# k-flouris/cmf

Hardware: AMD Instinct MI355X
Metric: log-density evals/sec (JtJ-cholesky path), MNIST D=784 d=64 bs=512 (higher is better)
Workload: dtype f32 (3x3 tangent convs as bf16x3 split MFMA, fp32 accumulate); 1 GPU; C3: MNIST-shaped (1,28,28) uint8-range + U[0,1) noise, non-square flow d=64, cholesky J^T J log-det + g_ij off-diagonal L1 + reconstruction, eval/no_grad; per_gpu_batch=512, global_batch=512, D=784, latent_dimension=64, parallelism=dp1

## Files before the change

cmf_amd/_lib.py:

```python
import ctypes as C
import os
import threading

_HERE = os.path.dirname(os.path.abspath(__file__))
LIB_PATH = os.path.join(_HERE, "libcmf_amd.so")

F_NONE, F_RELU, F_TANH, F_RAW, F_SELF_RELU, F_RELU_BITS = 0, 1, 2, 3, 4, 5
O_NONE, O_TANH, O_STANH = 0, 1, 2

_fp = C.c_void_p
_ll = C.c_longlong
_i = C.c_int
_f = C.c_float
_d = C.c_double


class ConvTangentArgs(C.Structure):
    _fields_ = [("x", _fp), ("x_np", _ll), ("x_ci", _ll), ("x_px", _ll),
                ("f", _fp), ("f_np", _ll), ("f_ci", _ll), ("f_px", _ll), ("fmode", _i),
                ("w", _fp),
                ("y", _fp), ("y_np", _ll), ("y_co", _ll), ("y_px", _ll),
                ("r", _fp), ("r_np", _ll), ("r_co", _ll), ("r_px", _ll),
                ("np", _i), ("cin", _i), ("cout", _i), ("H", _i), ("W", _i), ("nc", _i), ("taps", _i),
                ("bias", _fp), ("f_group", _i), ("x_sl", _ll), ("y_sl", _ll), ("r_sl", _ll),
                ("fo", _fp), ("fo_np", _ll), ("fo_co", _ll), ("fo_px", _ll), ("fomode", _i),
                ("mask_out", _fp), ("mask_np", _ll), ("amax_in", _fp), ("amax_out", _fp), ("live", _i),
                ("ymask", _fp), ("ymask_np", _ll),
                ("head_w", _fp), ("head_cout", _i), ("head_a", _fp), ("head_a_np", _ll), ("head_a_c", _ll), ("head_a_px", _ll),
                ("head_y", _fp), ("head_y_np", _ll), ("head_y_co", _ll), ("head_y_px", _ll),
                ("seed", _fp), ("seed_np", _ll), ("seed_col", _ll), ("seed_w", _fp)]


class ConvPrimalArgs(C.Structure):
    _fields_ = [("x", _fp), ("x_b", _ll), ("x_c", _ll), ("x_px", _ll),
                ("f", _fp), ("f_c", _ll), ("f_px", _ll), ("imode", _i),
                ("w", _fp), ("bias", _fp), ("sw", _fp), ("sb", _fp),
                ("y", _fp), ("y_b", _ll), ("y_c", _ll), ("y_px", _ll),
                ("g", _fp),
                ("r", _fp), ("r_b", _ll), ("r_c", _ll), ("r_px", _ll),
                ("omode", _i),
                ("B", _i), ("cin", _i), ("cout", _i), ("H", _i), ("W", _i), ("taps", _i)]


class ProbeApplyArgs(C.Structure):
    _fields_ = [("r", _fp), ("r_np", _ll), ("r_px", _ll),
                ("t", _fp), ("t_np", _ll), ("t_c", _ll), ("t_px", _ll),
                ("cls", _fp),
                ("y", _fp), ("y_np", _ll), ("y_px", _ll),
                ("ymask", _fp), ("ymask_np", _ll),
                ("np", _i), ("cin", _i), ("H", _i), ("W", _i), ("nc", _i), ("ns", _i)]


MLP_MAX_LAYERS = 8
WGRAD_MAX_BATCH = 16


class MlpCouplerArgs(C.Structure):
    _fields_ = [("z", _fp), ("z_b", _ll), ("t", _fp), ("t_f", _ll), ("w", _fp),
                ("zi", _fp), ("si", _fp), ("ti", _fp), ("n_mod", _i),
                ("B", _i), ("cin", _i), ("chan_off", _i), ("chan_step", _i), ("n_layers", _i),
                ("width", _i * (MLP_MAX_LAYERS + 1)), ("w_off", _ll * MLP_MAX_LAYERS), ("decode", _i), ("lj", _fp), ("ncols", _i)]


SIGNATURES = {
    "cmf_version": (C.c_char_p, []),
    "cmf_pack_weight": (_i, [_fp, _fp, _i, _i, _i, _i, C.POINTER(_ll), _fp]),
    "cmf_pack_weights_batched": (_i, [_fp, _i, _fp]),
    "cmf_conv_tangent": (_i, [C.POINTER(ConvTangentArgs), _fp]),
    "cmf_pack_weight_bf16x3": (_i, [_fp, _fp, _i, _i, C.POINTER(_ll), _fp]),
    "cmf_pack_weight_bf16x3_t": (_i, [_fp, _fp, _i, _i, _i, C.POINTER(_ll), _fp]),
    "cmf_conv_tangent_bf16x3": (_i, [C.POINTER(ConvTangentArgs), _fp]),
    "cmf_probe_apply": (_i, [C.POINTER(ProbeApplyArgs), _fp]),
    "cmf_pack_seed_weight": (_i, [_fp, _fp, _fp]),
    "cmf_seed_panel": (_i, [_fp, _ll, _ll, _fp, _fp, _ll, _ll, _i, _i, _i, _i, _fp]),
    "cmf_pack_weight_f16x3": (_i, [_fp, _fp, _i, _i, _i, C.POINTER(_ll), _fp]),
    "cmf_conv_tangent_f16x3": (_i, [C.POINTER(ConvTangentArgs), _fp]),
    "cmf_conv_tangent_f16x3_item": (_i, [C.POINTER(ConvTangentArgs), _i, _fp]),
    "cmf_absmax": (_i, [_fp, _ll, _fp, _fp]),
    "cmf_conv_tangent_wgrad_ws": (_ll, [C.POINTER(ConvTangentArgs)]),
    "cmf_conv_tangent_wgrad": (_i, [C.POINTER(ConvTangentArgs), _fp, _fp, _fp, _ll, _fp]),
    "cmf_conv_tangent_wgrad_bf16x3": (_i, [C.POINTER(ConvTangentArgs), _fp, _fp, _fp, _ll, _fp]),
    "cmf_conv_tangent_wgrad_bf16x3_batched": (_i, [C.POINTER(ConvTangentArgs), _i, C.POINTER(_fp), C.POINTER(_fp), C.POINTER(_fp), _fp, _ll, _fp]),
    "cmf_primal_regroup": (_i, [_fp, _fp, _i, _ll, _i, _fp]),
    "cmf_conv_primal": (_i, [C.POINTER(ConvPrimalArgs), _fp]),
    "cmf_acl_primal": (_i, [_fp, _ll, _fp, _ll, _fp, _fp, _fp, _i, _i, _i, _fp, _fp]),
    "cmf_acl_tangent": (_i, [_fp, _ll, _ll, _fp, _ll, _ll, _i, _fp, _ll, _fp, _ll, _fp, _fp, _fp, _fp, _i, _i, _fp]),
    "cmf_acl_cotangent": (_i, [_fp, _ll, _ll, _fp, _ll, _ll, _i, _fp, _ll, _fp, _ll, _fp, _fp, _fp, _fp, _i, _i, _fp]),
    "cmf_acl_primal_backward": (_i, [_fp, _ll, _fp, _ll, _fp, _ll, _fp, _fp, _fp, _fp, _i, _i, _i, _fp, _fp]),
    "cmf_acl_cross_terms": (_i, [_fp, _ll, _ll, _fp, _ll, _ll, _fp, _ll, _ll, _i, _fp, _ll, _fp, _ll, _fp, _fp, _fp, _fp, _i, _i,
                            _fp, _fp, _fp, _fp]),
    "cmf_gather_primal": (_i, [_fp, _ll, _fp, _ll, _fp, _i, _i, _fp]),
    "cmf_gather_tangent": (_i, [_fp, _ll, _ll, _fp, _ll, _ll, _fp, _i, _i, _i, _fp]),
    "cmf_seed_tangent": (_i, [_fp, _ll, _ll, _fp, _i, _i, _fp, _i, _i, _i, _fp]),
    "cmf_gram_cholesky": (_i, [_fp, _ll, _ll, _i, _i, _i, _i, _fp, _fp, _fp, _fp, _fp, _fp, _fp]),
    "cmf_cholesky_retry": (_i, [_fp, _i, _i, _i, _f, _fp, _fp, _fp, _fp, _fp]),
    "cmf_gram_condition": (_i, [_fp, _fp, _i, _i, _f, _fp, _fp, _fp, _fp, _fp]),
    "cmf_metric_stats_ws": (_ll, [_i, _i, _i, _i]),
    "cmf_metric_stats_accumulate": (_i, [_fp, _i, _i, _i, _fp, _fp, _ll, _fp, _fp]),
    "cmf_gram_spectrum": (_i, [_fp, _i, _i, _fp, _fp, _fp, _fp, _fp]),
    "cmf_gauss_newton_step": (_i, [_fp, _ll, _ll, _i, _i, _i, _i, _fp, _fp, _fp, _fp, _fp, _fp, _fp, _fp, _fp]),
    "cmf_stanh_backward": (_i, [_fp, _fp, _fp, _fp, _fp, _fp, _fp, _fp, _fp, _i, _i, _i, _fp]),
    "cmf_tanh_cross_terms": (_i, [_fp, _ll, _ll, _fp, _ll, _ll, _fp, _fp, _i, _i, _i, _fp]),
    "cmf_tanh_backward": (_i, [_fp, _fp, _fp, _ll, _fp, _fp]),
    "cmf_affine_prior_backward": (_i, [_fp, _ll, _fp, _ll, _fp, _i, _i, _fp, _fp, _fp, _fp]),
    "cmf_accumulate": (_i, [_fp, _fp, _ll, _fp]),
    "cmf_relu_bits": (_i, [_fp, _fp, _i, _i, _i, _fp]),
    "cmf_channel_sum": (_i, [_fp, _ll, _ll, _ll, _ll, _i, _i, _i, _i, _fp, _fp]),
# ... 120 lines not shown
```

cmf_amd/csrc/common.h:

```cpp
#pragma once
#include <hip/hip_runtime.h>
#include "cmf_amd.h"

typedef float f32x4 __attribute__((ext_vector_type(4)));

#define CMF_LAUNCH_CHECK()                         \
  do {                                             \
    hipError_t e_ = hipGetLastError();             \
    if (e_ != hipSuccess) return (int)e_;          \
  } while (0)

hipError_t cmf_set_dynamic_lds(const void* fn, int bytes);
int cmf_device_cus();

static inline int cmf_ceil_div(long long a, long long b) { return (int)((a + b - 1) / b); }

__device__ __forceinline__ float wave_sum(float v) {
#pragma unroll
  for (int o = 32; o > 0; o >>= 1) v += __shfl_xor(v, o, 64);
  return v;
}

__device__ __forceinline__ float block_sum(float v, float* red) {
  v = wave_sum(v);
  const int w = threadIdx.x >> 6, nw = (blockDim.x + 63) >> 6;
  __syncthreads();
  if ((threadIdx.x & 63) == 0) red[w] = v;
  __syncthreads();
  float t = 0.f;
  for (int i = 0; i < nw; ++i) t += red[i];
  return t;
}

int cmf_conv_head(const cmf_conv_tangent_args& a, hipStream_t s);

int cmf_wide_gram_cholesky(const float* t, long long t_b, long long t_r, int n_rows, int d, int B, float* jtj, float* logdet,
                           float* l1_off, float* l1_diag, int* info, int* fail, hipStream_t s);
int cmf_wide_cholesky_retry(float* jtj, int d, int B, int attempt, float eps, float* logdet, float* l1_diag, int* info, int* fail,
                            hipStream_t s);
int cmf_wide_gram_backward(const float* t, long long t_b, long long t_r, int n_rows, int nc, int d, int B, const float* jtj,
                           const float* g_logdet, const float* g_l1off, const float* g_l1diag, float* dt, long long dt_b,
                           long long dt_r, float* ws, hipStream_t s);
int cmf_wide_gram_backward_matrix(const float* t, long long t_b, long long t_r, int n_rows, int nc, int d, int B, const float* m,
                                  float* dt, long long dt_b, long long dt_r, hipStream_t s);
int cmf_wide_hutch_cg(const float* jtj, const float* eps, int d, int S, int B, int max_iter, int min_iter, float tol, float* u,
                      float* w, float* val, int* iters, hipStream_t s);
int cmf_wide_hutch_cotangent(const float* u, const float* eps, const float* w, int d, int S, int B, const float* g_val,
                             const float* g_off, const float* g_diag, float* M, hipStream_t s);
```

cmf_amd/csrc/conv_head.hip:

```cpp
#include <stdint.h>

#include "common.h"

namespace {

constexpr int HID = 64, KJ = HID * 9, NT = 192, ACC = 16;
constexpr int SLICE = HID * 16;

__device__ __forceinline__ int out_pixel(int po, int W, int live) {
  if (!live) return po;
  const int wh = W >> 1, row = po / wh, k = po - row * wh;
  return row * W + 2 * k + ((row + live - 1) & 1);
}

template <int CP>
__global__ __launch_bounds__(NT, CP == 8 ? 2 : 3) void conv_head_kernel(cmf_conv_tangent_args a, int n_out, int tiles_per_sample, int ntiles) {
  constexpr int P = ACC / CP;
  __shared__ __attribute__((aligned(16))) float Es[P * KJ * CP];
  __shared__ __attribute__((aligned(16))) float Gs[HID * ACC];
  __shared__ unsigned long long um[P * 9];
  __shared__ unsigned long long alv[P];
  __shared__ int pixs[P];

  const int per = (ntiles + 7) >> 3;
// ... 129 lines not shown
        for (int i = 0; i < n / 2; ++i) {
          const float mine = hi ? val[n / 2 + i] : val[i], send = hi ? val[i] : val[n / 2 + i];
          val[i] = mine + __shfl_xor(send, off, 64);
        }
      } else {
        val[0] += __shfl_xor(val[0], off, 64);
      }
    }
    float* yb = a.head_y + (long long)b * a.head_y_np + (long long)(p0 + p) * a.head_y_px + sl * 16 + (lane & 3) * 4;
    constexpr int KEEP = N >= 16 ? N / 16 : 1;
#pragma unroll
    for (int i = 0; i < KEEP; ++i) {
      const int idx = ((cl * N) >> 4) + i, o = idx >> 2;
      if (o < cout && (N >= 16 || !(lane & 4))) yb[(long long)o * a.head_y_co + (idx & 3)] = val[i];
    }
  }
}

template <int CP>
int launch(const cmf_conv_tangent_args& a, hipStream_t s) {
  constexpr int P = ACC / CP;
  const int n_out = a.live ? a.H * a.W / 2 : a.H * a.W;
  const long long tiles = (n_out + P - 1) / P, ntiles = tiles * a.np;
  if (ntiles > 0x7ffffff0LL) return CMF_ERANGE;
  const int grid = 8 * (int)((ntiles + 7) / 8);
  hipLaunchKernelGGL(conv_head_kernel<CP>, dim3(grid), dim3(NT), 0, s, a, n_out, (int)tiles, (int)ntiles);
  CMF_LAUNCH_CHECK();
  return 0;
}

}

int cmf_conv_head(const cmf_conv_tangent_args& a, hipStream_t s) {
  if (!a.x || !a.w || !a.f || !a.r || !a.head_w || !a.head_a || !a.head_y) return CMF_EINVAL;
  if (a.fmode != CMF_F_RELU_BITS || a.taps != 9 || a.cin != HID || a.cout != HID) return CMF_EINVAL;
  if (a.head_cout < 1 || a.head_cout > 8 || a.np <= 0 || a.H <= 0 || a.W <= 0 || a.nc <= 0 || a.nc % 16) return CMF_EINVAL;
  if (a.bias || a.fo || a.ymask || a.mask_out || a.live < 0 || a.live > 2 || (a.live && a.W % 2)) return CMF_EINVAL;
  if (!((a.W % 14 == 0 && a.H % 2 == 0) || (a.W % 8 == 0 && a.H % 4 == 0))) return CMF_EINVAL;
  const long long HW = (long long)a.H * a.W;
  if (HW > (1 << 24)) return CMF_ERANGE;
  if (a.x_ci != 16 || a.x_sl != SLICE || a.r_co != 16 || a.r_sl != SLICE) return CMF_EINVAL;
  if ((a.x_np | a.x_px | a.r_np | a.r_px | a.head_y_np | a.head_y_co | a.head_y_px) % 4) return CMF_EINVAL;
  if (a.x_px < (long long)HID * a.nc || a.r_px < (long long)HID * a.nc || a.head_y_px < a.nc) return CMF_EINVAL;
  if ((uintptr_t)a.x % 16 || (uintptr_t)a.r % 16 || (uintptr_t)a.head_y % 16 || (uintptr_t)a.w % 4 || (uintptr_t)a.head_w % 4) return CMF_EINVAL;
  if ((uintptr_t)a.f % 8 || a.f_np % 8 || a.f_np < HW * (HID / 8)) return CMF_EINVAL;
  const int cp = a.head_cout <= 2 ? 2 : a.head_cout <= 4 ? 4 : 8;
  return cp == 2 ? launch<2>(a, s) : cp == 4 ? launch<4>(a, s) : launch<8>(a, s);
}
```

cmf_amd/engine.py:

```python
import ctypes as C
import threading

import numpy as np
import torch
import torch.nn as nn

from . import _lib
from ._lib import (F_NONE, F_RELU, F_TANH, F_RAW, F_SELF_RELU, F_RELU_BITS, O_NONE, O_TANH, O_STANH, ConvPrimalArgs,
                   ConvTangentArgs)


def _stream():
    return C.c_void_p(torch.cuda.current_stream().cuda_stream)


def _p(t):
    return None if t is None else C.c_void_p(t.data_ptr())


def require_gpu(t, what="input"):
    if not t.is_cuda:
        raise RuntimeError(f"cmf_amd: {what} is on {t.device}; the log-density path runs only through the HIP "
                           "kernels on an AMD GPU (there is no CPU fallback)")
    if t.dtype != torch.float32:
# ... 346 lines not shown
                (lib.cmf_conv_tangent_bf16x3, "cmf_conv_tangent_bf16x3") if split else (lib.cmf_conv_tangent, "cmf_conv_tangent"))
    launch = lambda: _lib.check(fn(C.byref(a), _stream()), what)
    if f16 and item_channels:
        launch = lambda: _lib.check(lib.cmf_conv_tangent_f16x3_item(C.byref(a), int(item_channels), _stream()), "cmf_conv_tangent_f16x3_item")
    if fmode == F_SELF_RELU and not f16 and _lib.tracing():
        run = launch

        def launch():
            with _lib.role("primal"):
                run()
    TIMER = _timer()
    if TIMER is None:
        return launch()
    px_in = float(H) * W * nc * np_
    px = px_in * (0.5 if live else 1.0)
    TIMER.wrap(f"conv_tangent_t{taps}_ci{cin}_co{cout}" + ("_primal" if fmode == F_SELF_RELU else "_primal_bwd" if pbwd else "_live" if live else ""),
               2.0 * (cin + (1 if seed is not None else 0)) * cout * taps * px,
               4.0 * (px_in * cin + px * (cout + (cout if res_t is not None else 0))
                      + (float(seed["np"]) * np_ if seed is not None else 0.0)), launch)


def _conv_tangent_head(lib, a, x_t, x_off, x_np, x_ci, x_px, weight, taps, y_t, y_np, y_co, y_px, np_, cin, cout, H, W, nc, fmode, f,
                       f_np, res_t, res_off, res_np, x_sl, y_off, live, head):
    wf, act = head["weight"], head["act"]
    hc = int(wf.shape[0])
    w2, wf = weight.detach(), wf.detach().reshape(hc, -1)
    assert w2.is_contiguous() and wf.is_contiguous() and act.is_contiguous() and w2.dtype == wf.dtype == act.dtype == torch.float32
    a.x = C.c_void_p(x_t.data_ptr() + 4 * int(x_off)); a.x_np, a.x_ci, a.x_px, a.x_sl = int(x_np), int(x_ci), int(x_px), int(x_sl)
    a.f = _p(f); a.f_np = int(f_np); a.fmode = int(fmode)
    a.w = _p(w2)
    a.r = None if res_t is None else C.c_void_p(res_t.data_ptr() + 4 * int(res_off))
    a.r_np, a.r_co, a.r_px, a.r_sl = int(x_np if res_np is None else res_np), int(x_ci), int(x_px), int(x_sl)
    a.np, a.cin, a.cout, a.H, a.W, a.nc, a.taps, a.live = int(np_), int(cin), int(cout), int(H), int(W), int(nc), int(taps), int(live)
    a.head_w, a.head_cout = _p(wf), hc
    a.head_a = _p(act); a.head_a_np, a.head_a_c, a.head_a_px = int(cin) * H * W, H * W, 1
    a.head_y = C.c_void_p(y_t.data_ptr() + 4 * int(y_off)); a.head_y_np, a.head_y_co, a.head_y_px = int(y_np), int(y_co), int(y_px)
    launch = lambda: _lib.check(lib.cmf_conv_tangent_bf16x3(C.byref(a), _stream()), "cmf_conv_tangent_bf16x3")
    TIMER = _timer()
    if TIMER is None:
        return launch()
    px_out = float(H) * W * np_ * (0.5 if live else 1.0)
    TIMER.wrap(f"conv_tangent_t{taps}_ci{cin}_co{cout}" + ("_live" if live else ""),
               2.0 * hc * px_out * (cin * taps * cout + (cin * taps + cout) * nc),
               4.0 * (float(H) * W * np_ * nc * cin + px_out * (nc * cout + cout + nc * hc)), launch)


_WGRAD_WS = {}


def conv_tangent_wgrad(x_t, x_off, x_np, x_ci, x_px, gy_t, gy_off, y_np, y_co, y_px, dw, taps, np_, cin, cout, H, W, nc,
                       fmode=F_NONE, f=None, f_np=0, f_ci=0, f_px=0, f_group=1, x_sl=16, y_sl=16, precision=None):
    lib = _lib.load()
    assert dw.dtype == torch.float32 and dw.is_contiguous() and dw.numel() == cout * cin * taps
    a = ConvTangentArgs()
    a.x = C.c_void_p(x_t.data_ptr() + 4 * int(x_off)); a.x_np, a.x_ci, a.x_px = int(x_np), int(x_ci), int(x_px)
    fbits = isinstance(f, BitMask)
    if fbits:
        f, f_np, f_ci, f_px, fmode = f.data, f.np_bytes, 0, 0, F_RELU_BITS
    a.f = _p(f); a.f_np, a.f_ci, a.f_px = int(f_np), int(f_ci), int(f_px); a.fmode = fmode
    a.y_np, a.y_co, a.y_px = int(y_np), int(y_co), int(y_px)
    a.np, a.cin, a.cout, a.H, a.W, a.nc, a.taps = int(np_), int(cin), int(cout), int(H), int(W), int(nc), int(taps)
    a.f_group = int(f_group)
    a.x_sl, a.y_sl = int(x_sl), int(y_sl)
    need = int(lib.cmf_conv_tangent_wgrad_ws(C.byref(a)))
    key = (x_t.device, torch.cuda.current_stream().cuda_stream)
    ws = _WGRAD_WS.get(key)
    if ws is None or ws.numel() * 4 < need:
        ws = _WGRAD_WS[key] = torch.empty(need // 4, dtype=torch.float32, device=x_t.device)
    gy = C.c_void_p(gy_t.data_ptr() + 4 * int(gy_off))
    split = ((precision or cfg().tangent) == "bf16x3" and taps == 9 and cin % 64 == 0 and cout % 64 == 0 and nc % 32 == 0
             and fmode in (F_NONE, F_RELU, F_SELF_RELU, F_RELU_BITS) and f_group <= 1)
    assert not fbits or split, "bit-mask factors are read by the split-precision weight-gradient kernel only"
    fn, what = (lib.cmf_conv_tangent_wgrad_bf16x3, "cmf_conv_tangent_wgrad_bf16x3") if split else \
               (lib.cmf_conv_tangent_wgrad, "cmf_conv_tangent_wgrad")
# ... 898 lines not shown
    y = primal_regroup(yg.view(G, -1), False).view(B, cout, H, W)
    g = primal_regroup(gg.view(G, -1), False).view(B, cout, H, W)
    if not need_acts:
        return y, g, None
    std_of = lambda t: primal_regroup(t.view(G, -1), False).view(B, hid, H, W)
    if train:
        out = ActList([a0] + masks[:-1] + [std_of(acts[-1])] if bits else [a0] + [std_of(t) for t in acts[1:]])
        out.grouped = acts
        return y, g, out
    if bits:
        return y, g, [a0] + masks[:-1] + [std_of(acts[-1])]
    return y, g, [a0] + [std_of(t) for t in acts[1:]]


def _view_rows(T, view):
    if T.layout == "panel":
        HW = view.geom.HW
        rows = T.data[: T.B * T.N * T.nc].view(T.B, T.N // HW, HW * T.nc)[:, view.chan_off::view.chan_step][:, :view.cin]
        out = Tangent(T.B, view.cin * HW, T.nc, "panel", T.data.device)
    else:
        rows = T.data[: T.B * T.N * T.nc].view(T.N, T.B * T.nc)[view.chan_off::view.chan_step][:view.cin]
        out = Tangent(T.B, view.cin, T.nc, "fmajor", T.data.device)
    out.data.view(rows.shape).copy_(rows)
    return out


CHECKERBOARD_TAIL = True

SKIP_DEAD_ROWS = True

FOLD_HEAD = True


PROBE_FRONT = True

PROBE_FRONT_SHAPES = {(28, 28, 1)}

PROBE_CLASSES = 13

SEED_RESIDUAL = True


def probe_plan(mask):
    mask = np.asarray(mask)
    if mask.ndim != 3:
        return None
    cin, H, W = mask.shape
    if not 1 <= cin <= 2:
        return None
    r, col = np.meshgrid(np.arange(H), np.arange(W), indexing="ij")
    cls = (np.mod(r - 5 * col, 2 * PROBE_CLASSES) >> 1)[None] + PROBE_CLASSES * np.arange(cin)[:, None, None]
    cls = np.where(mask != 0, cls, -1).astype(np.int8)
    for r0 in range(H):
        for c0 in range(W):
            win = cls[:, max(r0 - 2, 0):r0 + 3, max(c0 - 2, 0):c0 + 3].reshape(-1)
            win = win[win >= 0]
            if len(np.unique(win)) != len(win):
                return None
    ns = (PROBE_CLASSES * cin + 15) // 16
    flat = cls.reshape(-1)
    probes = np.zeros((cin * H * W, 16 * ns), dtype=np.float32)
    rows = np.flatnonzero(flat >= 0)
    probes[rows, flat[rows]] = 1.0
    return {"cls": flat, "ns": ns, "probes": probes}


# ... 30 lines not shown
        launch()
    else:
        TIMER.wrap("seed_panel", 0.0, 4.0 * B * nc * (col + HW), launch)
    return dict(panel=out, np=nc * col, col=col)


def seed_pack_host(w):
    w = np.asarray(w, dtype=np.float32).reshape(64, 9)
    out = np.zeros((4, 64, 4), dtype=np.float32)
    for kq in range(3):
        for j in range(3):
            out[:, 16 * kq:16 * kq + 16, j] = w[:, 3 * kq + j].reshape(4, 16)
    return out


def seed_panel_index(H, W):
    idx = np.full(seed_plane(H, W), -1, dtype=np.int64)
    r, c = np.meshgrid(np.arange(H), np.arange(W), indexing="ij")
    idx[((r + 1) * (W + 2) + c + 1).reshape(-1)] = (r * W + c).reshape(-1)
    return idx


def _seed_pack(conv0, dev):
    def build():
        w = conv0.weight.detach().contiguous()
        assert tuple(w.shape) == (64, 1, 3, 3) and w.dtype == torch.float32
        out = torch.empty(4096, dtype=torch.uint8, device=dev)
        _lib.check(_lib.load().cmf_pack_seed_weight(_p(w), _p(out), _stream()), "cmf_pack_seed_weight")
        return out

    return DERIVED.get((id(conv0.weight), "seed-residual", str(dev)), [conv0.weight], build)


def _probe_hidden(conv0, view, plan, H, W, hid, dev):
    HW, ncp = H * W, 16 * plan["ns"]

    def build():
        out = torch.empty(HW * hid * ncp, dtype=torch.float32, device=dev)
        conv_tangent(plan["probes"], 0, view.cin * HW * ncp, HW * ncp, ncp, conv0.weight, 9, out, hid * HW * ncp, 16, hid * ncp,
                     1, view.cin, hid, H, W, ncp, fmode=F_RAW, f=view.mask, f_np=0, f_ci=HW, f_px=1, y_sl=hid * 16)
        return out

    return DERIVED.get((id(conv0.weight), "probe-front", H, W, view.cin, str(dev)), [conv0.weight], build)


def probe_front(conv0, conv1, T, view, plan, factor, ymask, scratch, u, H, W):
    B, nc, HW, hid, dev = T.B, T.nc, H * W, conv1.out_channels, T.data.device
    assert hid == 64 and T.layout == "panel"
    ncp = 16 * plan["ns"]
    conv_tangent(_probe_hidden(conv0, view, plan, H, W, hid, dev), 0, 0, 16, hid * ncp, conv1.weight, 9, scratch,
                 hid * HW * ncp, 16, hid * ncp, B, hid, hid, H, W, ncp, x_sl=hid * 16, y_sl=hid * 16, ymask=ymask, **factor)
    probe_apply(scratch, hid * HW * ncp, hid * ncp, T.data, view.chan_off * HW * nc, T.t_b, view.chan_step * HW * nc, nc,
                plan["cls"], u, hid * HW * nc, hid * nc, B, view.cin, H, W, nc, plan["ns"], ymask=ymask)


def net_tangent(net, T, view, acts, transpose_packs=False, save=None):
    geo, B, nc, dev = view.geom, T.B, T.nc, T.data.device
    if save is not None:
        save.append(_view_rows(T, view))
    if net.kind == "resnet":
        conv0, blocks, convf = _resnet_parts(net)
        hid, cout, H, W, HW = conv0.out_channels, convf.out_channels, geo.H, geo.W, geo.HW
        new = lambda c: Tangent(B, c * HW, nc, "panel", dev)
        pn = lambda c: (c * HW * nc, HW * nc, nc)
        hd = (hid * HW * nc, 16, hid * nc)
        hsl = hid * 16
        fg = getattr(acts, "f_group", 1)
        fs = dict(f_np=hid * HW * fg, f_ci=HW * fg, f_px=fg, f_group=fg)
        fk = lambda t: dict(fmode=F_RELU_BITS, f=t.data, f_np=t.np_bytes) if isinstance(t, BitMask) else dict(fmode=F_RELU, f=t, **fs)
        u, h2 = new(hid), new(hid)
        compact = (CHECKERBOARD_TAIL and view.live is not None and save is None and fg == 1 and len(blocks) > 0 and hid % 64 == 0
                   and W % 2 == 0 and _use_bf16x3(9, hid, W, False, H, hid))
        filt = SKIP_DEAD_ROWS and save is None and hid % 64 == 0 and _use_bf16x3(9, hid, W, False, H, hid)
        fold = (FOLD_HEAD and view.live is not None and save is None and fg == 1 and len(blocks) > 0 and hid == 64 and cout <= 8 and nc % 16 == 0
                and isinstance(acts[2 * len(blocks) - 1], BitMask) and _use_bf16x3(9, hid, W, False, H, hid))
        plan = getattr(view, "probe", None)
        probe = (PROBE_FRONT and plan is not None and save is None and fg == 1 and len(blocks) > 0 and hid == 64 and view.mask is not None
                 and T.layout == "panel" and nc % 16 == 0 and nc > 16 * plan["ns"] and (H, W, view.cin) in PROBE_FRONT_SHAPES
                 and cfg().tangent == "bf16x3" and _use_bf16x3(9, hid, W, False, H, hid))
        seeded = SEED_RESIDUAL and probe and view.cin == 1 and len(blocks) >= 2 and isinstance(acts[1], BitMask)
        h = None
        if not seeded:
            h = new(hid)
            conv_tangent(T.data, view.chan_off * HW * nc, T.t_b, view.chan_step * HW * nc, nc, conv0.weight, 9, h.data, *hd,
                         B, view.cin, hid, H, W, nc, fmode=F_RAW if view.mask is not None else F_NONE, f=view.mask, f_np=0,
                         f_ci=HW, f_px=1, y_sl=hsl)
        for k, blk in enumerate(blocks):
            a_in, c1 = acts[2 * k], acts[2 * k + 1]
            ym = c1 if filt and isinstance(c1, BitMask) else None
            if probe and k == 0:
                probe_front(conv0, blk.conv1, T, view, plan, fk(a_in), ym, h2.data, u.data, H, W)
            else:
                conv_tangent(h.data, 0, *hd, blk.conv1.weight, 9, u.data, *hd, B, hid, hid, H, W, nc, x_sl=hsl, y_sl=hsl, **fk(a_in),
                             ymask=ym)
            if seeded and k == 0:
                sd = seed_panel(T, view, H, W)
                conv_tangent(u.data, 0, *hd, blk.conv2.weight, 9, h2.data, *hd, B, hid, hid, H, W, nc, x_sl=hsl, y_sl=hsl,
                             seed=dict(sd, pack=_seed_pack(conv0, dev)), **fk(c1))
                h, h2 = h2, new(hid)
                continue
            if fold and k + 1 == len(blocks):
                HWo = HW // 2 if compact else HW
                yt = Tangent(B, cout * HWo, nc, "panel", dev)
                conv_tangent(u.data, 0, *hd, blk.conv2.weight, 9, yt.data, cout * HWo * nc, HWo * nc, nc, B, hid, hid, H, W, nc,
                             res_t=h.data, res_np=hd[0], x_sl=hsl, live=view.live["parity"] if compact else 0,
                             head=dict(weight=convf.weight, act=acts[-1]), **fk(c1))
                if compact:
                    yt.compact = True
                return yt
            if compact and k + 1 == len(blocks):
                HWc = HW // 2
                hc = Tangent(B, hid * HWc, nc, "panel", dev)
                conv_tangent(u.data, 0, *hd, blk.conv2.weight, 9, hc.data, hid * HWc * nc, 16, hid * nc, B, hid, hid, H, W, nc,
                             res_t=h.data, res_np=hd[0], x_sl=hsl, y_sl=hsl, live=view.live["parity"], **fk(c1))
                a_last = gather_primal(acts[-1], view.live["act_idx"], hid * HWc)
                yt = Tangent(B, cout * HWc, nc, "panel", dev)
                conv_tangent(hc.data, 0, hid * HWc * nc, 16, hid * nc, convf.weight, 1, yt.data, cout * HWc * nc, HWc * nc, nc, B, hid,
                             cout, H, W // 2, nc, fmode=F_RELU, f=a_last, x_sl=hsl, f_np=hid * HWc, f_ci=HWc, f_px=1)
                yt.compact = True
                return yt
            conv_tangent(u.data, 0, *hd, blk.conv2.weight, 9, h2.data, *hd, B, hid, hid, H, W, nc, res_t=h.data, x_sl=hsl,
                         y_sl=hsl, **fk(c1))
# ... 259 lines not shown
```

include/cmf_amd.h:

```cpp
#ifndef CMF_AMD_H
#define CMF_AMD_H

#ifdef __cplusplus
extern "C" {
#endif

#define CMF_EINVAL (-1)
#define CMF_ERANGE (-2)

#define CMF_F_NONE 0
#define CMF_F_RELU 1
#define CMF_F_TANH 2
#define CMF_F_RAW  3
#define CMF_F_SELF_RELU 4
#define CMF_F_RELU_BITS 5

#define CMF_O_NONE  0
#define CMF_O_TANH  1
#define CMF_O_STANH 2

const char* cmf_version(void);

int cmf_pack_weight(const float* w, float* out, int cout, int cin, int taps, int transpose,
                    long long* out_floats, void* stream);

typedef struct {
  const float* w; void* out; long long total;
  int cout, cin, taps, transpose, kind, reserved;
} cmf_pack_desc;
int cmf_pack_weights_batched(const cmf_pack_desc* table, int n, void* stream);

typedef struct {
  const float* x; long long x_np, x_ci, x_px;
  const float* f; long long f_np, f_ci, f_px;
  int fmode;
  const float* w;
  float* y;       long long y_np, y_co, y_px;
  const float* r; long long r_np, r_co, r_px;
  int np, cin, cout, H, W, nc, taps;
  const float* bias;
  int f_group;
  long long x_sl, y_sl, r_sl;
  const float* fo; long long fo_np, fo_co, fo_px; int fomode;
  void* mask_out; long long mask_np;
  const float* amax_in; float* amax_out;
  int live;
  const void* ymask; long long ymask_np;
  const float* head_w; int head_cout;
  const float* head_a; long long head_a_np, head_a_c, head_a_px;
  float* head_y; long long head_y_np, head_y_co, head_y_px;
  const float* seed; long long seed_np, seed_col; const void* seed_w;
} cmf_conv_tangent_args;
int cmf_conv_tangent(const cmf_conv_tangent_args* a, void* stream);

int cmf_pack_weight_bf16x3(const float* w, void* out, int cout, int cin, long long* out_bytes, void* stream);
int cmf_pack_weight_bf16x3_t(const float* w, void* out, int cout, int cin, int transpose, long long* out_bytes, void* stream);
int cmf_conv_tangent_bf16x3(const cmf_conv_tangent_args* a, void* stream);
int cmf_pack_seed_weight(const float* w, void* out, void* stream);
int cmf_seed_panel(const float* v, long long v_np, long long v_px, const float* mask, float* out, long long out_np, long long out_col,
                   int np, int H, int W, int nc, void* stream);

typedef struct {
  const float* r; long long r_np, r_px;
  const float* t; long long t_np, t_c, t_px;
  const signed char* cls;
  float* y;       long long y_np, y_px;
  const void* ymask; long long ymask_np;
  int np, cin, H, W, nc, ns;
} cmf_probe_apply_args;
int cmf_probe_apply(const cmf_probe_apply_args* a, void* stream);

int cmf_pack_weight_f16x3(const float* w, void* out, int cout, int cin, int transpose, long long* out_bytes, void* stream);
int cmf_conv_tangent_f16x3(const cmf_conv_tangent_args* a, void* stream);
int cmf_conv_tangent_f16x3_item(const cmf_conv_tangent_args* a, int item_channels, void* stream);
int cmf_absmax(const float* x, long long n, float* out, void* stream);

long long cmf_conv_tangent_wgrad_ws(const cmf_conv_tangent_args* a);
int cmf_conv_tangent_wgrad(const cmf_conv_tangent_args* a, const float* gy, float* dw, float* ws, long long ws_bytes,
                           void* stream);
int cmf_conv_tangent_wgrad_bf16x3(const cmf_conv_tangent_args* a, const float* gy, float* dw, float* ws, long long ws_bytes,
                                  void* stream);
#define CMF_WGRAD_MAX_BATCH 16
int cmf_conv_tangent_wgrad_bf16x3_batched(const cmf_conv_tangent_args* a, int nprob, const float* const* x, const float* const* gy,
                                          float* const* dw, float* ws, long long ws_bytes, void* stream);

typedef struct {
  const float* x; long long x_b, x_c, x_px;
  const float* f; long long f_c, f_px;
  int imode;
  const float* w; const float* bias;
  const float* sw; const float* sb;
// ... 134 lines not shown
```

Before: 1518 evals/s.

## Fold last residual block's two convs and head into one composed 5x5 kernel

Adds a kernel that folds the final residual block (conv1, ReLU mask, conv2, ReLU mask) together with the output head. For each output pixel it builds an effective 5x5 per-pixel composed kernel by backpropagating the head weights through conv2 and conv1 with bf16x3 MFMA, then applies that kernel directly to the block input tangent panel. This skips materialising the intermediate block tangents across all nc columns, which targets the bandwidth and FLOP cost of two full 64x64 tangent convolutions. In exchange it does per-pixel kernel construction work and more LDS use, and it is enabled only for the 28x28 shape with cout=2.

Result: faster. 1541 evals/s, median of 6 (+1.5%).

```diff
diff --git a/cmf_amd/_lib.py b/cmf_amd/_lib.py
--- a/cmf_amd/_lib.py
+++ b/cmf_amd/_lib.py
@@ -28,7 +28,8 @@
                 ("ymask", _fp), ("ymask_np", _ll),
                 ("head_w", _fp), ("head_cout", _i), ("head_a", _fp), ("head_a_np", _ll), ("head_a_c", _ll), ("head_a_px", _ll),
                 ("head_y", _fp), ("head_y_np", _ll), ("head_y_co", _ll), ("head_y_px", _ll),
-                ("seed", _fp), ("seed_np", _ll), ("seed_col", _ll), ("seed_w", _fp)]
+                ("seed", _fp), ("seed_np", _ll), ("seed_col", _ll), ("seed_w", _fp),
+                ("block_w1", _fp), ("block_m1", _fp), ("block_m1_np", _ll)]
 
 
 class ConvPrimalArgs(C.Structure):
@@ -73,6 +74,7 @@
     "cmf_probe_apply": (_i, [C.POINTER(ProbeApplyArgs), _fp]),
     "cmf_pack_seed_weight": (_i, [_fp, _fp, _fp]),
     "cmf_seed_panel": (_i, [_fp, _ll, _ll, _fp, _fp, _ll, _ll, _i, _i, _i, _i, _fp]),
+    "cmf_pack_block_weight": (_i, [_fp, _fp, C.POINTER(_ll), _fp]),
     "cmf_pack_weight_f16x3": (_i, [_fp, _fp, _i, _i, _i, C.POINTER(_ll), _fp]),
     "cmf_conv_tangent_f16x3": (_i, [C.POINTER(ConvTangentArgs), _fp]),
     "cmf_conv_tangent_f16x3_item": (_i, [C.POINTER(ConvTangentArgs), _i, _fp]),
diff --git a/cmf_amd/csrc/common.h b/cmf_amd/csrc/common.h
--- a/cmf_amd/csrc/common.h
+++ b/cmf_amd/csrc/common.h
@@ -33,6 +33,7 @@
 }
 
 int cmf_conv_head(const cmf_conv_tangent_args& a, hipStream_t s);
+int cmf_conv_block_head(const cmf_conv_tangent_args& a, hipStream_t s);
 
 int cmf_wide_gram_cholesky(const float* t, long long t_b, long long t_r, int n_rows, int d, int B, float* jtj, float* logdet,
                            float* l1_off, float* l1_diag, int* info, int* fail, hipStream_t s);
diff --git a/cmf_amd/csrc/conv_block_head.hip b/cmf_amd/csrc/conv_block_head.hip
--- /dev/null
+++ b/cmf_amd/csrc/conv_block_head.hip
@@ -0,0 +1,378 @@
+#include <stdint.h>
+
+#include "common.h"
+
+namespace {
+
+typedef __bf16 bf16x8 __attribute__((ext_vector_type(8)));
+typedef __bf16 bf16x2 __attribute__((ext_vector_type(2)));
+typedef float f32x2 __attribute__((ext_vector_type(2)));
+typedef unsigned u32x4 __attribute__((ext_vector_type(4)));
+
+constexpr int HID = 64, KJ = HID * 9, NT = 512, ROWS = 16, ND = 25, HALO = 8, XB = 4;
+constexpr int SLICE = HID * 16;
+static_assert(2 * KJ > 2 * NT && 2 * KJ <= 3 * NT && (2 * KJ - 2 * NT) % 64 == 0, "phase B: two units per thread, a third for whole waves");
+constexpr int W1_FRAGS = 9 * 4 * 2 * 2 * 64;
+
+__device__ __forceinline__ unsigned pack_hi(float a, float b, float& ra, float& rb) {
+  bf16x2 h = __builtin_convertvector(f32x2{a, b}, bf16x2);
+  const unsigned bits = __builtin_bit_cast(unsigned, h);
+  ra = a - __builtin_bit_cast(float, bits << 16);
+  rb = b - __builtin_bit_cast(float, bits & 0xffff0000u);
+  return bits;
+}
+__device__ __forceinline__ unsigned pack_lo(float a, float b) {
+  bf16x2 h = __builtin_convertvector(f32x2{a, b}, bf16x2);
+  return __builtin_bit_cast(unsigned, h);
+}
+
+__global__ void pack_block_weight_kernel(const float* __restrict__ w, u32x4* __restrict__ out) {
+  const int idx = blockIdx.x * 256 + threadIdx.x;
+  if (idx >= W1_FRAGS) return;
+  const int l = idx & 63, hl = (idx >> 6) & 1, ks = (idx >> 7) & 1, ct = (idx >> 8) & 3, t1 = idx >> 10;
+  const int c = 16 * ct + (l & 15), ci0 = 32 * ks + 8 * (l >> 4);
+  unsigned r[4];
+#pragma unroll
+  for (int jj = 0; jj < 4; ++jj) {
+    const float v0 = w[((ci0 + 2 * jj) * HID + c) * 9 + t1], v1 = w[((ci0 + 2 * jj + 1) * HID + c) * 9 + t1];
+    float ra, rb;
+    const unsigned h = pack_hi(v0, v1, ra, rb);
+    r[jj] = hl ? pack_lo(ra, rb) : h;
+  }
+  out[idx] = u32x4{r[0], r[1], r[2], r[3]};
+}
+
+struct Tile {
+  int row0, s0, xb, Ws, H, W, live;
+  __device__ __forceinline__ bool slot(int p, int& row, int& col, int& po) const {
+    const int s = s0 + (p & 1);
+    row = row0 + (p >> 1);
+    col = live ? 2 * s + ((row + live - 1) & 1) : s;
+    po = row * Ws + s;
+    return row < H && s < Ws;
+  }
+};
+
+__device__ __forceinline__ void load_w1(u32x4 (&b)[2][2], const u32x4* __restrict__ wp, int ct, int lane, int t1) {
+#pragma unroll
+  for (int ks = 0; ks < 2; ++ks)
+#pragma unroll
+    for (int hl = 0; hl < 2; ++hl) b[ks][hl] = wp[(((t1 * 4 + ct) * 2 + ks) * 2 + hl) * 64 + lane];
+}
+
+template <int HALF, int CP>
+__device__ __forceinline__ void build_half(const u32x4* __restrict__ wp, const u32x4* As, float* Ks, const float* Gs,
+                                           const unsigned long long* ha, const int* ctr, int ct, int lane) {
+  constexpr int D0 = HALF ? 12 : 0, NDH = HALF ? 13 : 12;
+  const f32x4 zero = {0.f, 0.f, 0.f, 0.f};
+  f32x4 acc[NDH];
+  u32x4 af[9][2][2], bw[2][2][2];
+#pragma unroll
+  for (int i = 0; i < NDH; ++i) acc[i] = zero;
+  load_w1(bw[0], wp, ct, lane, 0);
+#pragma unroll
+  for (int t2 = 0; t2 < 9; ++t2)
+#pragma unroll
+    for (int ks = 0; ks < 2; ++ks)
+#pragma unroll
+      for (int hl = 0; hl < 2; ++hl) af[t2][ks][hl] = As[((t2 * 2 + ks) * 2 + hl) * 64 + lane];
+#pragma unroll
+  for (int t1 = 0; t1 < 9; ++t1) {
+    if (t1 < 8) load_w1(bw[(t1 + 1) & 1], wp, ct, lane, t1 + 1);
+#pragma unroll
+    for (int t2 = 0; t2 < 9; ++t2) {
+      const int d = (t1 / 3 + t2 / 3) * 5 + t1 % 3 + t2 % 3;
+      if (d >= D0 && d < D0 + NDH) {
+#pragma unroll
+        for (int ks = 0; ks < 2; ++ks) {
+          const bf16x8 ah = __builtin_bit_cast(bf16x8, af[t2][ks][0]), al = __builtin_bit_cast(bf16x8, af[t2][ks][1]);
+          const bf16x8 bh = __builtin_bit_cast(bf16x8, bw[t1 & 1][ks][0]), bl = __builtin_bit_cast(bf16x8, bw[t1 & 1][ks][1]);
+          acc[d - D0] = __builtin_amdgcn_mfma_f32_16x16x32_bf16(al, bh, acc[d - D0], 0, 0, 0);
+          acc[d - D0] = __builtin_amdgcn_mfma_f32_16x16x32_bf16(ah, bl, acc[d - D0], 0, 0, 0);
+          acc[d - D0] = __builtin_amdgcn_mfma_f32_16x16x32_bf16(ah, bh, acc[d - D0], 0, 0, 0);
+        }
+      }
+    }
+  }
+  const int c = 16 * ct + (lane & 15);
+#pragma unroll
+  for (int dl = 0; dl < NDH; ++dl) {
+    const int d = D0 + dl;
+#pragma unroll
+    for (int i = 0; i < 4; ++i) {
+      const int row = 4 * (lane >> 4) + i, p = row / CP, o = row % CP;
+      const int at = ctr[p];
+      const bool on = at >= 0 && ((ha[at + (d / 5 - 2) * HALO + d % 5 - 2] >> c) & 1);
+      float v = on ? acc[dl][i] : 0.f;
+      if (d == 12) v = Gs[c * ROWS + row] + v;
+      Ks[((p * ND + d) * HID + c) * CP + o] = v;
+    }
+  }
+}
+
+template <int R, int CP>
+__device__ __forceinline__ void phase_b(const float* __restrict__ w2, const float* Gs, const unsigned long long* um, u32x4* As, int tid) {
+  int q[R], rh[R];
+  float acc[R][8];
+#pragma unroll
+  for (int r = 0; r < R; ++r) {
+    const int u = tid + r * NT;
+    rh[r] = u >= KJ, q[r] = u - rh[r] * KJ;
+#pragma unroll
+    for (int i = 0; i < 8; ++i) acc[r][i] = 0.f;
+  }
+#pragma unroll 8
+  for (int c = 0; c < HID; ++c) {
+    float w[R];
+#pragma unroll
+    for (int r = 0; r < R; ++r) w[r] = w2[c * KJ + q[r]];
+#pragma unroll
+    for (int r = 0; r < R; ++r) {
+      const f32x4 g0 = *reinterpret_cast<const f32x4*>(&Gs[c * ROWS + rh[r] * 8]), g1 = *reinterpret_cast<const f32x4*>(&Gs[c * ROWS + rh[r] * 8 + 4]);
+#pragma unroll
+      for (int k = 0; k < 4; ++k) {
+        acc[r][k] = fmaf(g0[k], w[r], acc[r][k]);
+        acc[r][4 + k] = fmaf(g1[k], w[r], acc[r][4 + k]);
+      }
+    }
+  }
+  unsigned short* A16 = reinterpret_cast<unsigned short*>(As);
+#pragma unroll
+  for (int r = 0; r < R; ++r) {
+    const int ci = q[r] / 9, tap = q[r] - ci * 9, ks = ci >> 5, kq = (ci >> 3) & 3, j = ci & 7;
+#pragma unroll
+    for (int i = 0; i < 8; ++i) {
+      const int row = rh[r] * 8 + i, p = row / CP;
+      const float e = ((um[p * 9 + tap] >> ci) & 1) ? acc[r][i] : 0.f;
+      float ra, rb;
+      const unsigned h = pack_hi(e, 0.f, ra, rb);
+      const unsigned l = pack_lo(ra, 0.f);
+      const int at = ((tap * 2 + ks) * 2 * 64 + kq * 16 + row) * 8 + j;
+      A16[at] = (unsigned short)(h & 0xffffu);
+      A16[at + 64 * 8] = (unsigned short)(l & 0xffffu);
+    }
+  }
+}
+
+template <int CP>
+__global__ __launch_bounds__(NT, 2) void conv_block_head_kernel(cmf_conv_tangent_args a, int tiles_x, int tiles_per_sample, int ntiles) {
+  constexpr int P = ROWS / CP, TR = P / 2 > 0 ? P / 2 : 1, PU = P / 2;
+  static_assert(P >= 2, "two output columns per tile");
+  __shared__ __attribute__((aligned(16))) float Ks[ROWS * ND * HID];
+  __shared__ __attribute__((aligned(16))) u32x4 As[9 * 2 * 2 * 64];
+  __shared__ __attribute__((aligned(16))) float Gs[HID * ROWS];
+  __shared__ unsigned long long um[P * 9];
+  __shared__ unsigned long long ha[HALO * HALO];
+  __shared__ unsigned long long hl[HALO * HALO];
+  __shared__ unsigned long long alv[P];
+  __shared__ int ctr[P];
+
+  const int per = (ntiles + 7) >> 3;
+  const int item = (int)(blockIdx.x & 7) * per + (int)(blockIdx.x >> 3);
+  if (item >= ntiles) return;
+  const int b = item / tiles_per_sample, tl = item - b * tiles_per_sample, ty = tl / tiles_x, tx = tl - ty * tiles_x;
+  const int tid = threadIdx.x, lane = tid & 63, wv = __builtin_amdgcn_readfirstlane(tid >> 6);
+  const int H = a.H, W = a.W, cout = a.head_cout;
+  Tile T;
+  T.H = H, T.W = W, T.live = a.live, T.Ws = a.live ? W >> 1 : W, T.row0 = ty * TR, T.s0 = 2 * tx, T.xb = a.live ? 4 * tx : 2 * tx;
+  const int y0 = T.row0 - 2, x0 = T.xb - 2;
+
+  if (tid < P * 9) {
+    const int p = tid / 9, tap = tid - p * 9;
+    int row, col, po;
+    unsigned long long m = 0;
+    if (T.slot(p, row, col, po)) {
+      const int r = row + tap / 3 - 1, c = col + tap % 3 - 1;
+      if (r >= 0 && r < H && c >= 0 && c < W)
+        m = *reinterpret_cast<const unsigned long long*>(reinterpret_cast<const unsigned char*>(a.block_m1) + (long long)b * a.block_m1_np +
+                                                         (long long)(r * W + c) * (HID / 8));
+    }
+    um[tid] = m;
+  } else if (tid >= 256 && tid < 256 + HALO * HALO) {
+    const int q = tid - 256, r = y0 + (q >> 3), c = x0 + (q & 7);
+    unsigned long long m = 0;
+    if (r >= 0 && r < H && c >= 0 && c < W)
+      m = *reinterpret_cast<const unsigned long long*>(reinterpret_cast<const unsigned char*>(a.f) + (long long)b * a.f_np +
+                                                       (long long)(r * W + c) * (HID / 8));
+    ha[q] = m;
+    hl[q] = m;
+  }
+  for (int p = wv; p < P; p += NT / 64) {
+    int row, col, po;
+    const bool ok = T.slot(p, row, col, po);
+    bool on = false;
+    if (ok) on = a.head_a[(long long)b * a.head_a_np + (long long)lane * a.head_a_c + (long long)(row * W + col) * a.head_a_px] > 0.f;
+    const unsigned long long bal = __ballot(on);
+    if (lane == 0) {
+      alv[p] = bal;
+      ctr[p] = ok ? (row - y0) * HALO + (col - x0) : -1;
+    }
+#pragma unroll
+    for (int o = 0; o < CP; ++o) Gs[(lane * P + p) * CP + o] = (on && o < cout) ? a.head_w[o * HID + lane] : 0.f;
+  }
+  __syncthreads();
+  if (tid < P) {
+    int row, col, po;
+    if (T.slot(tid, row, col, po)) hl[ctr[tid]] |= alv[tid];
+  }
+
+  if (wv < (2 * KJ - 2 * NT) / 64)
+    phase_b<3, CP>(a.w, Gs, um, As, tid);
+  else
+    phase_b<2, CP>(a.w, Gs, um, As, tid);
+  __syncthreads();
+
+  {
+    const u32x4* wp = reinterpret_cast<const u32x4*>(a.block_w1);
+    if (wv < 4)
+      build_half<0, CP>(wp, As, Ks, Gs, ha, ctr, wv & 3, lane);
+    else
+      build_half<1, CP>(wp, As, Ks, Gs, ha, ctr, wv & 3, lane);
+  }
+  __syncthreads();
+
+  const int nsl = a.nc >> 4, cl = lane >> 2;
+  const f32x4 zero = {0.f, 0.f, 0.f, 0.f};
+  for (int unit = wv; unit < nsl * 2; unit += NT / 64) {
+    const int sl = unit >> 1, ph = unit & 1;
+    int prow[PU], pcol[PU], ppo[PU];
+    bool pok[PU];
+    int ylo = H, yhi = -1, xlo = W, xhi = -1;
+#pragma unroll
+    for (int k = 0; k < PU; ++k) {
+      pok[k] = T.slot(ph * PU + k, prow[k], pcol[k], ppo[k]);
+      if (pok[k]) {
+        ylo = min(ylo, prow[k] - 2), yhi = max(yhi, prow[k] + 2);
+        xlo = min(xlo, pcol[k] - 2), xhi = max(xhi, pcol[k] + 2);
+      }
+    }
+    if (yhi < 0) continue;
+    ylo = max(ylo, 0), yhi = min(yhi, H - 1), xlo = max(xlo, 0), xhi = min(xhi, W - 1);
+    const float* hb = a.x + (long long)b * a.x_np + sl * SLICE + lane * 4;
+    f32x4 acc[PU][CP];
+#pragma unroll
+    for (int k = 0; k < PU; ++k)
+#pragma unroll
+      for (int o = 0; o < CP; ++o) acc[k][o] = zero;
+
+    for (int y = ylo; y <= yhi; ++y) {
+#pragma unroll 1
+      for (int xs = xlo; xs <= xhi; xs += XB) {
+        f32x4 v[XB][4];
+#pragma unroll
+        for (int xi = 0; xi < XB; ++xi) {
+#pragma unroll
+          for (int ch = 0; ch < 4; ++ch) v[xi][ch] = zero;
+          const int x = xs + xi;
+          if (x <= xhi) {
+            const unsigned long long m = hl[(y - y0) * HALO + (x - x0)];
+            const float* src = hb + (long long)(y * W + x) * a.x_px;
+#pragma unroll
+            for (int ch = 0; ch < 4; ++ch)
+              if ((m >> (ch * 16 + cl)) & 1) v[xi][ch] = *reinterpret_cast<const f32x4*>(src + ch * 256);
+          }
+        }
+#pragma unroll
+        for (int xi = 0; xi < XB; ++xi) {
+          const int x = xs + xi;
+#pragma unroll
+          for (int k = 0; k < PU; ++k) {
+            const int dy = y - prow[k] + 2, dx = x - pcol[k] + 2;
+            if (x <= xhi && pok[k] && dy >= 0 && dy < 5 && dx >= 0 && dx < 5) {
+              const float* coef = &Ks[(((ph * PU + k) * ND + dy * 5 + dx) * HID + cl) * CP];
+#pragma unroll
+              for (int ch = 0; ch < 4; ++ch) {
+                const float* e4 = static_cast<const float*>(__builtin_assume_aligned(coef + ch * 16 * CP, CP < 4 ? 8 : 16));
+#pragma unroll
+                for (int o = 0; o < CP; ++o) {
+                  const float e = e4[o];
+#pragma unroll
+                  for (int q = 0; q < 4; ++q) acc[k][o][q] = fmaf(e, v[xi][ch][q], acc[k][o][q]);
+                }
+              }
+            }
+          }
+        }
+      }
+    }
+
+    constexpr int N = 4 * CP;
+#pragma unroll
+    for (int k = 0; k < PU; ++k) {
+      float val[N];
+#pragma unroll
+      for (int o = 0; o < CP; ++o)
+#pragma unroll
+        for (int q = 0; q < 4; ++q) val[4 * o + q] = acc[k][o][q];
+#pragma unroll
+      for (int s = 0; s < 4; ++s) {
+        const int off = 32 >> s, n = N >> s;
+        if (n >= 2) {
+          const bool hi = lane & off;
+#pragma unroll
+          for (int i = 0; i < n / 2; ++i) {
+            const float mine = hi ? val[n / 2 + i] : val[i], send = hi ? val[i] : val[n / 2 + i];
+            val[i] = mine + __shfl_xor(send, off, 64);
+          }
+        } else {
+          val[0] += __shfl_xor(val[0], off, 64);
+        }
+      }
+      if (pok[k]) {
+        float* yb = a.head_y + (long long)b * a.head_y_np + (long long)ppo[k] * a.head_y_px + sl * 16 + (lane & 3) * 4;
+        constexpr int KEEP = N >= 16 ? N / 16 : 1;
+#pragma unroll
+        for (int i = 0; i < KEEP; ++i) {
+          const int idx = ((cl * N) >> 4) + i, o = idx >> 2;
+          if (o < cout && (N >= 16 || !(lane & 4))) yb[(long long)o * a.head_y_co + (idx & 3)] = val[i];
+        }
+      }
+    }
+  }
+}
+
+template <int CP>
+int launch(const cmf_conv_tangent_args& a, hipStream_t s) {
+  constexpr int P = ROWS / CP, TR = P / 2;
+  const int Ws = a.live ? a.W / 2 : a.W;
+  const long long tiles_x = (Ws + 1) / 2, tiles = tiles_x * ((a.H + TR - 1) / TR), ntiles = tiles * a.np;
+  if (ntiles > 0x7ffffff0LL) return CMF_ERANGE;
+  const int grid = 8 * (int)((ntiles + 7) / 8);
+  hipLaunchKernelGGL(conv_block_head_kernel<CP>, dim3(grid), dim3(NT), 0, s, a, (int)tiles_x, (int)tiles, (int)ntiles);
+  CMF_LAUNCH_CHECK();
+  return 0;
+}
+
+}
+
+extern "C" int cmf_pack_block_weight(const float* w, void* out, long long* out_bytes, void* stream) {
+  if (!out) {
+    if (!out_bytes) return CMF_EINVAL;
+    *out_bytes = (long long)W1_FRAGS * 16;
+    return 0;
+  }
+  if (!w || (uintptr_t)out % 16 || (uintptr_t)w % 4) return CMF_EINVAL;
+  hipLaunchKernelGGL(pack_block_weight_kernel, dim3((W1_FRAGS + 255) / 256), dim3(256), 0, (hipStream_t)stream, w, (u32x4*)out);
+  CMF_LAUNCH_CHECK();
+  return 0;
+}
+
+int cmf_conv_block_head(const cmf_conv_tangent_args& a, hipStream_t s) {
+  if (!a.x || !a.w || !a.f || !a.block_w1 || !a.block_m1 || !a.head_w || !a.head_a || !a.head_y) return CMF_EINVAL;
+  if (a.r && a.r != a.x) return CMF_EINVAL;
+  if (a.fmode != CMF_F_RELU_BITS || a.taps != 9 || a.cin != HID || a.cout != HID) return CMF_EINVAL;
+  if (a.head_cout < 1 || a.head_cout > 8 || a.np <= 0 || a.H <= 0 || a.W <= 0 || a.nc <= 0 || a.nc % 16) return CMF_EINVAL;
+  if (a.bias || a.fo || a.ymask || a.mask_out || a.seed || a.live < 0 || a.live > 2 || (a.live && a.W % 2)) return CMF_EINVAL;
+  if (!((a.W % 14 == 0 && a.H % 2 == 0) || (a.W % 8 == 0 && a.H % 4 == 0))) return CMF_EINVAL;
+  const long long HW = (long long)a.H * a.W;
+  if (HW > (1 << 24)) return CMF_ERANGE;
+  if (a.x_ci != 16 || a.x_sl != SLICE) return CMF_EINVAL;
+  if ((a.x_np | a.x_px | a.head_y_np | a.head_y_co | a.head_y_px) % 4) return CMF_EINVAL;
+  if (a.x_px < (long long)HID * a.nc || a.head_y_px < a.nc) return CMF_EINVAL;
+  if ((uintptr_t)a.x % 16 || (uintptr_t)a.head_y % 16 || (uintptr_t)a.w % 4 || (uintptr_t)a.head_w % 4 || (uintptr_t)a.block_w1 % 16)
+    return CMF_EINVAL;
+  if ((uintptr_t)a.f % 8 || a.f_np % 8 || a.f_np < HW * (HID / 8)) return CMF_EINVAL;
+  if ((uintptr_t)a.block_m1 % 8 || a.block_m1_np % 8 || a.block_m1_np < HW * (HID / 8)) return CMF_EINVAL;
+  const int cp = a.head_cout <= 2 ? 2 : a.head_cout <= 4 ? 4 : 8;
+  return cp == 2 ? launch<2>(a, s) : cp == 4 ? launch<4>(a, s) : launch<8>(a, s);
+}
diff --git a/cmf_amd/csrc/conv_head.hip b/cmf_amd/csrc/conv_head.hip
--- a/cmf_amd/csrc/conv_head.hip
+++ b/cmf_amd/csrc/conv_head.hip
@@ -185,6 +185,7 @@
 }
 
 int cmf_conv_head(const cmf_conv_tangent_args& a, hipStream_t s) {
+  if (a.block_w1) return cmf_conv_block_head(a, s);
   if (!a.x || !a.w || !a.f || !a.r || !a.head_w || !a.head_a || !a.head_y) return CMF_EINVAL;
   if (a.fmode != CMF_F_RELU_BITS || a.taps != 9 || a.cin != HID || a.cout != HID) return CMF_EINVAL;
   if (a.head_cout < 1 || a.head_cout > 8 || a.np <= 0 || a.H <= 0 || a.W <= 0 || a.nc <= 0 || a.nc % 16) return CMF_EINVAL;
diff --git a/cmf_amd/engine.py b/cmf_amd/engine.py
--- a/cmf_amd/engine.py
+++ b/cmf_amd/engine.py
@@ -402,6 +402,11 @@
     a.r = None if res_t is None else C.c_void_p(res_t.data_ptr() + 4 * int(res_off))
     a.r_np, a.r_co, a.r_px, a.r_sl = int(x_np if res_np is None else res_np), int(x_ci), int(x_px), int(x_sl)
     a.np, a.cin, a.cout, a.H, a.W, a.nc, a.taps, a.live = int(np_), int(cin), int(cout), int(H), int(W), int(nc), int(taps), int(live)
+    blk = head.get("conv1")
+    if blk is not None:
+        assert res_t is None and isinstance(blk["mask"], BitMask), "the folded block reads h as x and takes relu'(c1) from a BitMask"
+        a.block_w1 = _p(_block_pack(blk["weight"], x_t.device))
+        a.block_m1, a.block_m1_np = _p(blk["mask"].data), int(blk["mask"].np_bytes)
     a.head_w, a.head_cout = _p(wf), hc
     a.head_a = _p(act); a.head_a_np, a.head_a_c, a.head_a_px = int(cin) * H * W, H * W, 1
     a.head_y = C.c_void_p(y_t.data_ptr() + 4 * int(y_off)); a.head_y_np, a.head_y_co, a.head_y_px = int(y_np), int(y_co), int(y_px)
@@ -410,6 +415,10 @@
     if TIMER is None:
         return launch()
     px_out = float(H) * W * np_ * (0.5 if live else 1.0)
+    if blk is not None:
+        return TIMER.wrap(f"conv_tangent_t{taps}_ci{cin}_co{cout}" + ("_live" if live else ""),
+                          2.0 * hc * px_out * (cin * taps * cout + 3 * taps * cin * taps * cout + 25 * cout * nc),
+                          4.0 * (float(H) * W * np_ * (nc * cin + 4) + px_out * (cout + nc * hc)), launch)
     TIMER.wrap(f"conv_tangent_t{taps}_ci{cin}_co{cout}" + ("_live" if live else ""),
                2.0 * hc * px_out * (cin * taps * cout + (cin * taps + cout) * nc),
                4.0 * (float(H) * W * np_ * nc * cin + px_out * (nc * cout + cout + nc * hc)), launch)
@@ -1374,6 +1383,10 @@
 FOLD_HEAD = True
 
 
+FOLD_BLOCK = True
+
+FOLD_BLOCK_SHAPES = ((28, 28, 2),)
+
 PROBE_FRONT = True
 
 PROBE_FRONT_SHAPES = {(28, 28, 1)}
@@ -1470,6 +1483,19 @@
     return DERIVED.get((id(conv0.weight), "seed-residual", str(dev)), [conv0.weight], build)
 
 
+def _block_pack(weight, dev):
+    def build():
+        w = weight.detach().contiguous()
+        assert tuple(w.shape) == (64, 64, 3, 3) and w.dtype == torch.float32
+        n = C.c_longlong(0)
+        _lib.check(_lib.load().cmf_pack_block_weight(None, None, C.byref(n), None), "pack size")
+        out = torch.empty(n.value, dtype=torch.uint8, device=dev)
+        _lib.check(_lib.load().cmf_pack_block_weight(_p(w), _p(out), None, _stream()), "cmf_pack_block_weight")
+        return out
+
+    return DERIVED.get((id(weight), "fold-block", str(dev)), [weight], build)
+
+
 def _probe_hidden(conv0, view, plan, H, W, hid, dev):
     HW, ncp = H * W, 16 * plan["ns"]
 
@@ -1512,6 +1538,9 @@
         filt = SKIP_DEAD_ROWS and save is None and hid % 64 == 0 and _use_bf16x3(9, hid, W, False, H, hid)
         fold = (FOLD_HEAD and view.live is not None and save is None and fg == 1 and len(blocks) > 0 and hid == 64 and cout <= 8 and nc % 16 == 0
                 and isinstance(acts[2 * len(blocks) - 1], BitMask) and _use_bf16x3(9, hid, W, False, H, hid))
+        nb = len(blocks)
+        fold_block = (FOLD_BLOCK and fold and nb >= 2 and isinstance(acts[2 * nb - 2], BitMask) and isinstance(acts[2 * nb - 1], BitMask)
+                      and (H, W, cout) in FOLD_BLOCK_SHAPES)
         plan = getattr(view, "probe", None)
         probe = (PROBE_FRONT and plan is not None and save is None and fg == 1 and len(blocks) > 0 and hid == 64 and view.mask is not None
                  and T.layout == "panel" and nc % 16 == 0 and nc > 16 * plan["ns"] and (H, W, view.cin) in PROBE_FRONT_SHAPES
@@ -1526,6 +1555,15 @@
         for k, blk in enumerate(blocks):
             a_in, c1 = acts[2 * k], acts[2 * k + 1]
             ym = c1 if filt and isinstance(c1, BitMask) else None
+            if fold_block and k + 1 == nb:
+                HWo = HW // 2 if compact else HW
+                yt = Tangent(B, cout * HWo, nc, "panel", dev)
+                conv_tangent(h.data, 0, *hd, blk.conv2.weight, 9, yt.data, cout * HWo * nc, HWo * nc, nc, B, hid, hid, H, W, nc,
+                             x_sl=hsl, live=view.live["parity"] if compact else 0,
+                             head=dict(weight=convf.weight, act=acts[-1], conv1=dict(weight=blk.conv1.weight, mask=c1)), **fk(a_in))
+                if compact:
+                    yt.compact = True
+                return yt
             if probe and k == 0:
                 probe_front(conv0, blk.conv1, T, view, plan, fk(a_in), ym, h2.data, u.data, H, W)
             else:
diff --git a/include/cmf_amd.h b/include/cmf_amd.h
--- a/include/cmf_amd.h
+++ b/include/cmf_amd.h
@@ -50,6 +50,7 @@
   const float* head_a; long long head_a_np, head_a_c, head_a_px;
   float* head_y; long long head_y_np, head_y_co, head_y_px;
   const float* seed; long long seed_np, seed_col; const void* seed_w;
+  const void* block_w1; const void* block_m1; long long block_m1_np;
 } cmf_conv_tangent_args;
 int cmf_conv_tangent(const cmf_conv_tangent_args* a, void* stream);
 
@@ -57,6 +58,7 @@
 int cmf_pack_weight_bf16x3_t(const float* w, void* out, int cout, int cin, int transpose, long long* out_bytes, void* stream);
 int cmf_conv_tangent_bf16x3(const cmf_conv_tangent_args* a, void* stream);
 int cmf_pack_seed_weight(const float* w, void* out, void* stream);
+int cmf_pack_block_weight(const float* w, void* out, long long* out_bytes, void* stream);
 int cmf_seed_panel(const float* v, long long v_np, long long v_px, const float* mask, float* out, long long out_np, long long out_col,
                    int np, int H, int W, int nc, void* stream);
 
```
